# Jordy-VL/multi-modal-early-exit

Hardware: AMD Instinct MI355X
Metric: docs_per_sec (higher is better)
Workload: dtype f32 (operands split into 2 x f16, 3 f16 MFMA terms per MAC, f32 accumulate)

## Files before the change

include/mmee.h:

```cpp
#ifndef MMEE_H
#define MMEE_H

#include <stddef.h>
#include <stdint.h>

#ifdef __cplusplus
extern "C" {
#endif

#define MMEE_ABI_VERSION 4
#define MMEE_MAX_ENCODER_EXITS 64

enum { MMEE_EXIT_VISION_AVG = 0, MMEE_EXIT_TEXT_AVG = 1, MMEE_EXIT_TEXT_VISUAL_CONCAT = 2 };
enum { MMEE_STRATEGY_RAMP = 0, MMEE_STRATEGY_GATE = 1 };
enum { MMEE_CRIT_MAX_CONFIDENCE = 0, MMEE_CRIT_ENTROPY = 1, MMEE_CRIT_PATIENCE = 2, MMEE_CRIT_MARGIN = 3 };
enum { MMEE_RULE_PLAIN = 0, MMEE_RULE_STREAK = 1, MMEE_RULE_EITHER = 2 };
enum { MMEE_ARCH_LAYOUTLMV3 = 0, MMEE_ARCH_BEIT = 1 };
enum { MMEE_PREC_F32 = 0, MMEE_PREC_BF16 = 1, MMEE_PREC_F32_SPLIT = 2 };
enum { MMEE_DT_F32 = 0, MMEE_DT_F16 = 1, MMEE_DT_BF16 = 2 };
enum {
    MMEE_FLAG_DENSE_ROWS = 1,
    MMEE_FLAG_NO_EXIT = 2,
    MMEE_FLAG_WHOLE_LAYERS = 4,
    MMEE_FLAG_PROBE_ALWAYS = 8,
// ... 201 lines not shown
int ee_preprocess_images(const uint8_t* images, const void* desc, int32_t B, int32_t R, int32_t max_h, void* workspace,
                         size_t workspace_bytes, float* pixel_values, uint8_t* resized_u8, void* stream);
size_t ee_preprocess_workspace_bytes(int32_t B, int32_t R, int32_t max_h);
int ee_collate_pad(const int64_t* ids, const int64_t* boxes, const int64_t* offsets, int32_t B, int32_t T, int64_t pad_id,
                   int64_t* out_ids, int64_t* out_mask, int64_t* out_bbox, void* stream);

int ee_profile(ee_handle* h, int32_t enable);
int ee_profile_read(ee_handle* h, int32_t idx, char* name_out, int32_t name_cap, double* total_ms, int32_t* launches);

int ee_debug_gemm(const float* A, const float* W, const float* bias, const float* resid, float* Cout, int32_t M, int32_t N,
                  int32_t K, int32_t epi, int32_t wgs_per_cu, const int32_t* row_src, uint64_t* clk_probe, void* stream);

int ee_debug_gemm_split(const float* A, const float* W, const float* bias, const float* resid, float* Cout, int32_t M, int32_t N,
                        int32_t K, int32_t epi, int32_t out_split, float a_scale, float w_scale, float out_scale,
                        const int32_t* row_src, int32_t rows_A, int32_t iters, float* ms_out, void* stream);

#define MMEE_ATTN_KERNEL_F32 0
#define MMEE_ATTN_KERNEL_PAIR 1
#define MMEE_ATTN_KERNEL_IDX 2
#define MMEE_ATTN_KERNEL_IDX_NOBIAS 3
int ee_debug_attention(const float* qkv, int32_t qkv_rows, const int32_t* doc_off, int32_t n_docs, const int32_t* qkv_doc_off, const int32_t* pos,
                       const int32_t* x0, const int32_t* y1, const int32_t* masked, const float* w1, const float* wx, const float* wy, int32_t heads,
                       int32_t bins1, int32_t bins2, int32_t max_rel_pos, int32_t max_rel_2d_pos, int32_t max_pos, int32_t max_coord, int32_t kernel,
                       int32_t use_queue, int32_t q_limit, int32_t terms, void* ctx, int32_t* err_flag_out, void* stream);

typedef struct ee_debug_embed_args {
    const int64_t *input_ids, *attention_mask, *bbox, *position_ids, *token_type_ids;
    int32_t B, T, G, pad_id, vocab, max_2d, max_pos, type_vocab, dense_rows, H, cs, ss;
    const float *word, *type, *pos, *xtab, *ytab, *htab, *wtab, *inputs_embeds;
    const float *text_ln_g, *text_ln_b, *vis_ln_g, *vis_ln_b, *ln2_g, *ln2_b;
// ... 90 lines not shown
```

multi-modal-early-exit_amd/capi.py:

```python
from __future__ import annotations

import ctypes as C
import os
from typing import Optional

ABI_VERSION = 4
MAX_ENCODER_EXITS = 64
EXIT_KIND = {"vision_avg": 0, "text_avg": 1, "text_visual_concat": 2}
FLAG_DENSE_ROWS = 1
FLAG_NO_EXIT = 2
FLAG_WHOLE_LAYERS = 4
FLAG_PROBE_ALWAYS = 8
FLAG_XPROBE = 16
FLAG_ONE_TERM = 32
FLAG_LOW_LATENCY = 64
FLAG_STREAM_RESULTS = 128
CRIT_MAX_CONFIDENCE, CRIT_ENTROPY, CRIT_PATIENCE, CRIT_MARGIN = 0, 1, 2, 3
RULE_PLAIN, RULE_STREAK, RULE_EITHER = 0, 1, 2
SEARCH_GRID, SEARCH_SAMPLED, SEARCH_MIXTURES = 0, 1, 2
SEARCH_REFERENCE, SEARCH_POLICY = 0, 1
(METRIC_ACCURACY, METRIC_BRIER, METRIC_NLL, METRIC_F1_MICRO, METRIC_F1_MACRO, METRIC_ECE, METRIC_AURC, METRIC_AVG_CONF,
 METRIC_COUNT) = range(9)
DT_F32, DT_F16, DT_BF16 = 0, 1, 2
CLOCK_STAMP_WORDS = 4096
# ... 116 lines not shown
    "ee_rule_scan": (C.c_int, [_vp, C.c_double, _vp, _i32, _i32, _i32, C.POINTER(C.c_double), C.POINTER(_i32), _i32, _vp, _vp, _vp, _vp, _vp]),
    "ee_rule_sweep": (C.c_int, [_vp, _vp, _vp, _i32, _i32, _i32, _vp, _i32, C.POINTER(_i32), _i32, _i32, _vp, _vp, _vp, _vp]),
    "ee_patience_sweep": (C.c_int, [_vp, _vp, _i32, _i32, _i32, _vp, _i32, _vp, _vp, _vp, _vp]),
    "ee_pack_results": (C.c_int, [_vp, _vp, _vp, _i32, _i32, _vp, _vp]),
    "ee_unpack_results": (C.c_int, [_vp, _i32, _i32, _vp, _vp, _vp, _vp]),
    "ee_threshold_sweep": (C.c_int, [_vp, _vp, _i32, _i32, _vp, _i32, _vp, _vp, _vp, _vp]),
    "ee_threshold_search": (C.c_int, [_vp, _vp, _i32, _i32, _i32, _i32, C.c_int64, C.c_uint64, _vp, _i32, _vp, _vp, _vp, _vp, _vp, _vp, _vp, _vp, _vp]),
    "ee_threshold_search_cost": (C.c_int, [_vp, _vp, _vp, _i32, _i32, _i32, _i32, C.c_int64, C.c_uint64, _vp, _i32, _vp, _vp, _vp, _vp, _vp, _vp, _vp, _vp,
                                           _vp, _vp, _vp]),
    "ee_msp_table": (C.c_int, [_vp, _vp, _i32, _i32, _i32, _vp, _vp, _vp]),
    "ee_csf_table": (C.c_int, [_vp, _vp, _i32, _i32, _i32, _i32, _vp, _vp, _vp]),
    "ee_exit_metrics": (C.c_int, [_vp, _vp, _vp, _vp, _vp, _vp, _i32, _i32, _i32, _i32, _vp, _vp, _vp, _vp]),
    "ee_debug_gemm": (C.c_int, [_vp, _vp, _vp, _vp, _vp, _i32, _i32, _i32, _i32, _i32, _vp, _vp, _vp]),
    "ee_debug_gemm_split": (C.c_int, [_vp, _vp, _vp, _vp, _vp, _i32, _i32, _i32, _i32, _i32, C.c_float, C.c_float, C.c_float, _vp,
                                      _i32, _i32, C.POINTER(C.c_float), _vp]),
    "ee_debug_attn_stamps": (C.c_int, [_vp]),
    "ee_debug_attention": (C.c_int, [_vp, _i32, _vp, _i32, _vp, _vp, _vp, _vp, _vp, _vp, _vp, _vp, _i32, _i32, _i32, _i32, _i32, _i32, _i32, _i32,
                                     _i32, _i32, _i32, _vp, C.POINTER(_i32), _vp]),
    "ee_debug_prep": (C.c_int, [_vp, _vp, _vp, _vp, _vp, _i32, _i32, _i32, _i32, _i32, _i32, _i32, _i32, _i32, _vp, _vp, _vp, _vp, _vp, _vp, _vp, _vp,
                                C.POINTER(_i32), _vp]),
    "ee_debug_embed": (C.c_int, [C.POINTER(DebugEmbedArgs), C.POINTER(_i32), _vp]),
    "ee_debug_ln_rows": (C.c_int, [_vp, _vp, _vp, _vp, _i32, _i32, _vp, _vp, C.c_float, _vp, C.c_float, _i32, C.c_size_t, _vp, _vp, _vp, C.c_float,
                                   C.POINTER(_i32), _vp]),
    "ee_debug_xprobe": (C.c_int, [C.POINTER(DebugXProbeArgs), C.POINTER(_i32), _vp]),
    "ee_debug_head_out": (C.c_int, [C.POINTER(DebugHeadOutArgs), _vp]),
    "ee_debug_exit_decide": (C.c_int, [C.POINTER(DebugExitDecideArgs), _vp]),
    "ee_debug_rows_out": (C.c_int, [C.POINTER(DebugRowsOutArgs), _vp]),
    "ee_temperature_fit": (C.c_int, [_vp, _vp, _i32, _i32, _i32, _i32, _vp, _vp, _vp, _vp, _vp, _vp]),
    "ee_head_fit": (C.c_int, [_vp, _vp, _i32, _i32, _i32, _i32, C.c_double, C.c_double, _i32, _i32, _vp, C.c_size_t, _vp, _vp, _vp, _vp, _vp, _vp,
                              _vp, _vp, _vp]),
# ... 76 lines not shown
```

multi-modal-early-exit_amd/csrc/capi_tools.hip:

```cpp
#include <math.h>
#include <string.h>

#include <vector>

#include "capi_debug.h"

using namespace mmee;
using namespace mmee::capi;

namespace {

template <typename T>
struct TempUpload {
    T* dev = nullptr;
    hipStream_t s;
    const char* err = nullptr;
    TempUpload(const T* host, size_t n, hipStream_t stream) : s(stream) {
        if (hipMallocAsync((void**)&dev, sizeof(T) * n, s) != hipSuccess) { dev = nullptr; err = "hipMallocAsync failed"; }
        else if (hipMemcpyAsync(dev, host, sizeof(T) * n, hipMemcpyHostToDevice, s) != hipSuccess) err = "host-to-device copy failed";
    }
    TempUpload(const TempUpload&) = delete;
    ~TempUpload() { if (dev) (void)hipFreeAsync(dev, s); }
};

// ... 379 lines not shown
        launch_gemm_f32(g, epi, AMODE_ROWS, M, cus, reinterpret_cast<hipStream_t>(stream));
        set_gemm_wgs_per_cu(0);
    }
    return launch_status(nullptr, "ee_debug_gemm");
}

int ee_debug_attn_stamps(uint64_t* out8) {
    unsigned long long* d = mmee::attention_idx_stamps() ? mmee::attention_idx_stamps() : mmee::attention_pair_stamps();
    if (!out8 || !d) return fail(nullptr, "ee_debug_attn_stamps: no stamped launch has run (set MMEE_ATTN_STAMPS=1 before the first forward)");
    if (hipDeviceSynchronize() != hipSuccess || hipMemcpy(out8, d, 64, hipMemcpyDeviceToHost) != hipSuccess)
        return fail(nullptr, "ee_debug_attn_stamps: copy failed");
    (void)hipMemset(d, 0, 64);
    return 0;
}

int ee_debug_gemm_split(const float* A, const float* W, const float* bias, const float* resid, float* Cout, int32_t M, int32_t N,
                        int32_t K, int32_t epi, int32_t out_split, float a_scale, float w_scale, float out_scale,
                        const int32_t* row_src, int32_t rows_A, int32_t iters, float* ms_out, void* stream) {
    const int dbg = epi >> 4;
    epi &= 15;
#ifndef MMEE_DIAG
    if (dbg) return fail(nullptr, "ee_debug_gemm_split: timing variants (wrong results) exist in the diagnostic library only (make diag)");
#endif
    if (!A || !W || !Cout || M < 1 || rows_A < 1 || !mmee::gemm_split_supports(N, K) || epi < 0 || epi > 3 || iters < 1)
        return fail(nullptr, "ee_debug_gemm_split: bad argument (N %% 256, K %% 32)");
    if (epi == EPI_RESID && !resid) return fail(nullptr, "ee_debug_gemm_split: residual epilogue without a residual");
    hipStream_t s = reinterpret_cast<hipStream_t>(stream);
    const int cus = device_cus("ee_debug_gemm_split");
    if (!cus) return 1;
    float *As = nullptr, *Ws = nullptr;
    int* heads = nullptr;
    if (hipMalloc((void**)&As, (size_t)rows_A * K * 4) != hipSuccess || hipMalloc((void**)&Ws, (size_t)N * K * 4) != hipSuccess ||
        hipMalloc((void**)&heads, 512) != hipSuccess) {
        (void)hipFree(As); (void)hipFree(Ws); (void)hipFree(heads);
        return fail(nullptr, "ee_debug_gemm_split: hipMalloc failed");
    }
    mmee::launch_split_rows(A, As, nullptr, rows_A, rows_A, K, a_scale, cus, s);
    mmee::launch_split_rows(W, Ws, nullptr, N, N, K, w_scale, cus, s);
    GemmArgs g{};
    g.A = As; g.lda = K; g.W = Ws; g.bias = bias; g.C = Cout; g.ldc = N; g.resid = resid; g.ldr = N; g.m_static = M; g.N = N; g.K = K;
    g.scale = 1.f; g.alpha = 1.0f / (a_scale * w_scale); g.out_split = out_split ? 1 : 0; g.out_scale = out_scale;
    g.row_src = row_src; g.resid_row_src = row_src; g.tile_counter = heads; g.dbg_noload = dbg;
    unsigned long long* clk = nullptr;
    const int n_clk = 2 * 2 * cus;
    if (dbg && ms_out) {
        if (hipMalloc((void**)&clk, n_clk * 8) == hipSuccess) (void)hipMemsetAsync(clk, 0, n_clk * 8, s);
        g.clk_probe = clk;
    }
    hipEvent_t e0, e1;
    (void)hipEventCreate(&e0);
    (void)hipEventCreate(&e1);
    (void)hipMemsetAsync(heads, 0, 512, s);
    launch_gemm_split(g, epi, M, cus, s);
    (void)hipEventRecord(e0, s);
    for (int i = 1; i < iters; ++i) {
        (void)hipMemsetAsync(heads, 0, 512, s);
        launch_gemm_split(g, epi, M, cus, s);
// ... 3 lines not shown
    float ms = 0.f;
    if (iters > 1) (void)hipEventElapsedTime(&ms, e0, e1);
    if (ms_out) *ms_out = iters > 1 ? ms / (float)(iters - 1) : 0.f;
    if (clk) {
        std::vector<unsigned long long> hc(n_clk);
        (void)hipMemcpy(hc.data(), clk, n_clk * 8, hipMemcpyDeviceToHost);
        double sum = 0;
        int n = 0;
        for (int i = 0; i + 1 < n_clk; i += 2)
            if (hc[i + 1]) { sum += (double)hc[i] / (double)hc[i + 1] * 0.1; ++n; }
        ms_out[1] = n ? (float)(sum / n) : 0.f;
        (void)hipFree(clk);
    }
    (void)hipEventDestroy(e0);
    (void)hipEventDestroy(e1);
    (void)hipFree(As); (void)hipFree(Ws); (void)hipFree(heads);
    if (err != hipSuccess || hipGetLastError() != hipSuccess) return fail(nullptr, "ee_debug_gemm_split: launch failed: %s", hipGetErrorString(err));
    return 0;
}

}
```

multi-modal-early-exit_amd/csrc/gemm_split.hip:

```cpp
#include <cstdlib>
#include "mmee_common.h"

#include "gemm_split_kernel.h"

namespace mmee {

bool gemm_split_supports(int N, int K) { return N > 0 && K > 0 && N % 256 == 0 && K % 32 == 0; }

void launch_split_ffn_up(const GemmArgs& a, int max_m, int num_cus, hipStream_t s);

void launch_gemm_split(const GemmArgs& a_in, int epi, int max_m, int num_cus, hipStream_t s) {
    GemmArgs a = a_in;
    a.tile_order = a.N <= 768 ? 1 : 0;
    if (a.probe) a.terms = 3;
    if (a.probe) {
        if (a.out_split && epi == EPI_GELU) { launch_split_one<CfgP, EPI_GELU, true, false, 1>(a, max_m, num_cus, s); return; }
        if (!a.out_split && epi == EPI_RESID) { launch_split_one<CfgP, EPI_RESID, false, false, 1>(a, max_m, num_cus, s); return; }
        if (!a.out_split && epi == EPI_BIAS) { launch_split_one<CfgP, EPI_BIAS, false, false, 1>(a, max_m, num_cus, s); return; }
        if (!a.out_split && epi == EPI_TANH) { launch_split_one<CfgP, EPI_TANH, false, false, 1>(a, max_m, num_cus, s); return; }
    }
    if (a.k_splits > 1 && !a.out_split && epi == EPI_BIAS && a.terms != 1) {
        a.tile_counter = nullptr;
        launch_split_one<CfgP, EPI_BIAS, false, false, 1>(a, max_m, num_cus, s);
        return;
    }
    a.k_splits = 1;
    if (a.terms != 1 && (long)((max_m + 255) / 256) * (a.N / 256) * 2 <= (long)num_cus) {
        a.tile_counter = nullptr;
        if (a.out_split && epi == EPI_GELU) { launch_split_one<CfgP, EPI_GELU, true, false, 1>(a, max_m, num_cus, s); return; }
        if (a.out_split && epi == EPI_BIAS) { launch_split_one<CfgP, EPI_BIAS, true, false, 1>(a, max_m, num_cus, s); return; }
        if (!a.out_split && epi == EPI_RESID) { launch_split_one<CfgP, EPI_RESID, false, false, 1>(a, max_m, num_cus, s); return; }
        if (!a.out_split && epi == EPI_BIAS) { launch_split_one<CfgP, EPI_BIAS, false, false, 1>(a, max_m, num_cus, s); return; }
        if (!a.out_split && epi == EPI_TANH) { launch_split_one<CfgP, EPI_TANH, false, false, 1>(a, max_m, num_cus, s); return; }
        a.tile_counter = a_in.tile_counter;
    }
#ifdef MMEE_DIAG
    static const int order_env = diag_env_int("MMEE_GEMM_ORDER", -1);
    if (order_env == 0 || order_env == 1) a.tile_order = order_env;
    else if (order_env == 2) a.tile_order = a.N <= 768 ? 1 : 0;
    else if (order_env == 3 || order_env == 4) a.tile_order = a.N >= 2304 ? order_env - 1 : a.tile_order;
    static const int forced = diag_env_int("MMEE_SPLIT_CFG", 0);
    const bool use_a = forced == 1;
// ... 132 lines not shown
```

multi-modal-early-exit_amd/csrc/gemm_split_kernel.h:

```cpp
#pragma once
#include <cstdlib>
#include "mmee_common.h"

namespace mmee {


template <int BM_, int BN_, int ROWB_, int NST_, int WM_, int WN_, int WGS_, int MF_ = 32>
struct SplitCfg {
    static constexpr int BM = BM_, BN = BN_, ROWB = ROWB_, NST = NST_, WM = WM_, WN = WN_, WGS = WGS_;
    static constexpr int MF = MF_;
    static_assert(MF == 32 || (MF == 16 && ROWB == 128), "the 16x16x32 MFMA consumes one 128-byte row (k = 32) per step");
    static constexpr int NW = WM * WN, THREADS = NW * 64;
    static constexpr int KSTAGE = ROWB / 4;
    static constexpr int PROWS = 1024 / ROWB;
    static constexpr int PA = BM / PROWS / NW, PW = BN / PROWS / NW;
    static constexpr int PP = PA + PW;
    static constexpr int A_BYTES = BM * ROWB, STAGE_BYTES = (BM + BN) * ROWB, LOOP_BYTES = NST * STAGE_BYTES;
    static constexpr int EPI_BYTES = NW * 32 * 64 * 4;
    static_assert(BM == WM * 64 && BN == WN * 64, "one 64x64 sub-tile per wave");
    static_assert(PA * PROWS * NW == BM && PW * PROWS * NW == BN && PA >= 1 && PW >= 1, "DMA pieces must tile the stage");
    static_assert(EPI_BYTES <= LOOP_BYTES, "epilogue staging must fit in the stage ring");
    static_assert(NST >= 2 && NST <= 4, "ring depth");
    static_assert(THREADS <= 1024, "a workgroup is at most 16 waves");
    static_assert(WGS * (LOOP_BYTES + 16) <= 160 * 1024, "LDS budget of a CU (160 KiB) for WGS workgroups");
    static_assert(WGS * NW <= 32, "wave slots of a CU");
};
using CfgA = SplitCfg<128, 256, 64, 3, 2, 4, 2>;
using CfgB = SplitCfg<256, 256, 128, 2, 4, 4, 1>;
using CfgC = SplitCfg<256, 256, 128, 2, 4, 4, 1, 16>;
using CfgP = SplitCfg<128, 128, 128, 3, 2, 2, 1, 16>;


__device__ __forceinline__ void dma_piece(unsigned voff, unsigned long long base, unsigned lds_addr) {
    unsigned keep;
    asm volatile("s_mov_b32 %0, m0\n\ts_mov_b32 m0, %2\n\ts_nop 0\n\tglobal_load_lds_dwordx4 %1, %3\n\ts_mov_b32 m0, %0"
                 : "=&s"(keep)
                 : "v"(voff), "s"(lds_addr), "s"(base)
                 : "memory");
}

template <int EPI, bool OUT_SPLIT, int WN>
__device__ __forceinline__ void split_store_tile(const GemmArgs& g, float* smem, f32x16 (&acc)[2][2], int m0, int n0, int M,
                                                 int wave, int lane) {
    const int wr = wave / WN, wc = wave % WN;
    const int l31 = lane & 31, hh = lane >> 5;
    float* stg = smem + wave * (32 * 64);
    const int c4 = (lane & 15) * 4;
    const int col = n0 + wc * 64 + c4;
    f32x4 bv = f32x4{0.f, 0.f, 0.f, 0.f};
    if (g.bias) bv = *reinterpret_cast<const f32x4*>(g.bias + col);
    const float sc = (col < g.scale_cols) ? g.scale : 1.0f;
    f32x4 lam = f32x4{1.f, 1.f, 1.f, 1.f};
    if (g.col_scale) lam = *reinterpret_cast<const f32x4*>(g.col_scale + col);
// ... 53 lines not shown
                    const int c0 = __builtin_amdgcn_mov_dpp(h2.x, 0xDD, 0xf, 0xf, true), c1 = __builtin_amdgcn_mov_dpp(h2.y, 0xDD, 0xf, 0xf, true);
                    const int d0 = __builtin_amdgcn_mov_dpp(l2.x, 0xDD, 0xf, 0xf, true), d1 = __builtin_amdgcn_mov_dpp(l2.y, 0xDD, 0xf, 0xf, true);
                    piece.x = take_lo ? b0 : a0;
                    piece.y = take_lo ? b1 : a1;
                    piece.z = take_lo ? d0 : c0;
                    piece.w = take_lo ? d1 : c1;
                }
                if (row < M)
                    *reinterpret_cast<int4*>(reinterpret_cast<char*>(g.C) + (size_t)row * g.ldc * 4 + (size_t)(col >> 4) * 64 + (lane & 3) * 16) = piece;
            }
        }
    }
    if (OUT_SPLIT) split_flag_overflow(amax, g.err_flag);
}

template <int EPI, bool OUT_SPLIT, int WN, int RB>
__device__ __forceinline__ void split_store_tile16(const GemmArgs& g, float* smem, f32x4 (&acc)[4][4], int m0, int n0, int M,
                                                   int wave, int lane, const f32x4 bv, const f32x4 lam, const size_t c_shift = 0) {
    const int wr = wave / WN, wc = wave % WN;
    const int l15 = lane & 15, gq = lane >> 4;
    float* stg = smem + wave * (RB * 64);
    const int c4 = (lane & 15) * 4;
    const int col = n0 + wc * 64 + c4;
    const float sc = (col < g.scale_cols) ? g.scale : 1.0f;
    const float s_out = OUT_SPLIT ? g.out_scale : 1.0f;
    constexpr bool ACT = EPI == EPI_GELU || EPI == EPI_TANH;
    const bool sc_p2 = (__float_as_uint(sc) & 0x007fffffu) == 0u;
    const float fold = ACT ? 1.0f : s_out * (sc_p2 ? sc : 1.0f);
    const float post = ACT ? sc : (sc_p2 ? 1.0f : sc);
    const bool need_post = __builtin_amdgcn_readfirstlane((int)__float_as_uint(post)) != 0x3f800000;
    const bool need_lam = g.col_scale != nullptr;
    const float alpha_e = g.alpha * fold;
    const f32x4 be = bv * fold;
// ... 4 lines not shown
#pragma unroll
        for (int m2 = 0; m2 < RB / 16; ++m2)
#pragma unroll
            for (int ni = 0; ni < 4; ++ni)
#pragma unroll
                for (int e = 0; e < 4; ++e) {
                    const int r = 16 * m2 + 4 * gq + e;
                    stg[r * 64 + ((ni * 16 + l15) ^ (16 * (gq & 1)))] = acc[(RB / 16) * half + m2][ni][e];
                }
        asm volatile("" ::: "memory");
        const int rbase = m0 + wr * 64 + half * RB + (lane >> 4);
#pragma unroll
        for (int j = 0; j < RB / 4; ++j) {
            const int rl = (lane >> 4) + 4 * j;
            const int row = rbase + 4 * j;
            f32x4 v = *reinterpret_cast<const f32x4*>(stg + rl * 64 + (c4 ^ (16 * ((rl >> 2) & 1))));
#pragma unroll
            for (int t = 0; t < 4; t += 2) {
                f32x2 x = __builtin_elementwise_fma(f32x2{v[t], v[t + 1]}, (f32x2)(alpha_e), f32x2{be[t], be[t + 1]});
                if (need_post) x = x * (f32x2)(post);
                if (EPI == EPI_GELU) x = gelu_scaled2(x, gelu_c0, gelu_hs);
                if (EPI == EPI_TANH) { x[0] = tanhf(x[0]) * s_out; x[1] = tanhf(x[1]) * s_out; }
                if (need_lam) x = x * f32x2{lam[t], lam[t + 1]};
                v[t] = x[0];
                v[t + 1] = x[1];
            }
            if (row < M) {
                if (EPI == EPI_RESID) {
                    const int rs = g.resid_row_src ? g.resid_row_src[row] : row;
                    if (g.resid_split_inv != 0.f) {
                        const f32x4 r = load_split4_sum(g.resid + (size_t)rs * g.ldr, col);
#pragma unroll
                        for (int t = 0; t < 4; t += 2) {
                            const f32x2 y = __builtin_elementwise_fma(f32x2{r[t], r[t + 1]}, (f32x2)(g.resid_split_inv), f32x2{v[t], v[t + 1]});
                            v[t] = y[0];
                            v[t + 1] = y[1];
                        }
                    } else {
                        v += *reinterpret_cast<const f32x4*>(g.resid + (size_t)rs * g.ldr + col);
                    }
                }
                if (!OUT_SPLIT) *reinterpret_cast<f32x4*>(g.C + c_shift + (size_t)row * g.ldc + col) = v;
            }
// ... 60 lines not shown
    const int swz_even = ROWB == 64 ? ((p_row >> 2) & 3) : ((p_row >> 1) & 7);
    const unsigned chunk_even = 16u * (unsigned)(p_chunk ^ swz_even);
    const unsigned chunk_odd = ROWB == 64 ? chunk_even : 16u * (unsigned)(p_chunk ^ ((swz_even + 4) & 7));
    const unsigned rswz = ROWB == 64 ? (unsigned)((l31 >> 2) & 3) : (unsigned)((l31 >> 1) & 7);
    const unsigned a_row = (unsigned)(wr * 64 + l31) * ROWB;
    const unsigned w_row = (unsigned)A_BYTES + (unsigned)(wc * 64 + l31) * ROWB;
    const int l15 = lane & 15, lq = lane >> 4;
    const unsigned swz16 = (unsigned)((l15 >> 1) & 7);
    const unsigned c16_hi = 16u * (((unsigned)(lq & 1) + 4u * (unsigned)(lq >> 1)) ^ swz16);
    const unsigned c16_lo = 16u * (((unsigned)(lq & 1) + 4u * (unsigned)(lq >> 1) + 2u) ^ swz16);
    const unsigned a_row16 = (unsigned)(wr * 64 + l15) * ROWB;
    const unsigned w_row16 = (unsigned)A_BYTES + (unsigned)(wc * 64 + l15) * ROWB;
    const char* sbytes = reinterpret_cast<const char*>(smem);

    constexpr bool HANDOVER = Cfg::MF == 16 && NST == 2 && Cfg::NW * 4096 <= STAGE_BYTES;

    auto pop = [&](int& tm, int& tn) __attribute__((always_inline)) -> bool {
        if (g.tile_counter) {
            while (q_try < 8) {
                const int q = (my_xcd + q_try) & 7;
                if (tid == 0) *q_slot = atomicAdd(g.tile_counter + 16 * q, 1);
                __syncthreads();
                const int j = *q_slot;
                __syncthreads();
                if (g.tile_order >= 2) {
                    const int gq = q < n_groups ? (n_groups - q + 7) / 8 : 0;
                    if (g.tile_order == 2) {
                        constexpr int CW = 4;
                        const int nfull = tiles_n / CW, per_cb = gq * GM * CW;
                        int cb, jj, w;
// ... 35 lines not shown
                    continue;
                }
                ++q_try;
            }
            return false;
        }
        if (tile >= n_tiles) return false;
        int t2 = tile;
        if (KSPLIT) { t2 = tile / ksp; ks_pop = tile - t2 * ksp; }
        tm = t2 / tiles_n;
        tn = t2 - tm * tiles_n;
        tile += gridDim.x;
        return true;
    };

    struct TileCtx {
        int m0, n0;
        int kt0;
        unsigned a_voff[PA], w_voff[PW];
        unsigned long long a_base, w_base;
    };
    auto setup = [&](int tm, int tn, TileCtx& t) __attribute__((always_inline)) {
        t.m0 = __builtin_amdgcn_readfirstlane(tm * BM);
        t.n0 = __builtin_amdgcn_readfirstlane(tn * BN);
        t.kt0 = KSPLIT ? __builtin_amdgcn_readfirstlane(ks_pop * nk) : 0;
        int first = g.row_src ? g.row_src[t.m0] : t.m0;
        if (DIAG && (dbg & 16)) first = 0;
#pragma unroll
        for (int j = 0; j < PA; ++j) {
            const int piece = wave + Cfg::NW * j;
            int ra = t.m0 + Cfg::PROWS * piece + p_row;
            ra = ra < M ? ra : M - 1;
            if (DIAG && (dbg & 16)) ra = Cfg::PROWS * piece + p_row;
            const int sa = g.row_src ? g.row_src[ra] : ra;
            t.a_voff[j] = (unsigned)(sa - first) * (unsigned)g.lda * 4u + ((piece & 1) ? chunk_odd : chunk_even);
        }
#pragma unroll
        for (int j = 0; j < PW; ++j) {
            const int piece = wave + Cfg::NW * j;
            t.w_voff[j] = (unsigned)(Cfg::PROWS * piece + p_row) * (unsigned)g.K * 4u + ((piece & 1) ? chunk_odd : chunk_even);
        }
        const unsigned long long a_base_v = (unsigned long long)(size_t)g.A + (unsigned long long)first * (unsigned)g.lda * 4ull;
        const unsigned long long w_base_v = (unsigned long long)(size_t)g.W + (unsigned long long)t.n0 * (unsigned)g.K * 4ull;
        t.a_base = ((unsigned long long)(unsigned)__builtin_amdgcn_readfirstlane((int)(a_base_v >> 32)) << 32) |
                   (unsigned)__builtin_amdgcn_readfirstlane((int)(a_base_v & 0xffffffffu));
        t.w_base = ((unsigned long long)(unsigned)__builtin_amdgcn_readfirstlane((int)(w_base_v >> 32)) << 32) |
                   (unsigned)__builtin_amdgcn_readfirstlane((int)(w_base_v & 0xffffffffu));
    };
    auto issue = [&](const TileCtx& t, int kt, int buf) __attribute__((always_inline)) {
        const unsigned long long koff = (unsigned long long)(kt + (KSPLIT ? t.kt0 : 0)) * (unsigned)ROWB;
        const unsigned dst = lds0 + (unsigned)buf * STAGE_BYTES + (unsigned)wave * 1024u;
#pragma unroll
        for (int j = 0; j < PA; ++j) dma_piece(t.a_voff[j], t.a_base + koff, dst + (unsigned)(Cfg::NW * j) * 1024u);
#pragma unroll
        for (int j = 0; j < PW; ++j) dma_piece(t.w_voff[j], t.w_base + koff, dst + A_BYTES + (unsigned)(Cfg::NW * j) * 1024u);
    };

    TileCtx cur;
    int buf0 = 0;
    {
        int tm, tn;
        if (!pop(tm, tn)) return;
// ... 28 lines not shown
                asm volatile("s_waitcnt vmcnt(0)" ::: "memory");
            } else if (dbg & 4) {
                asm volatile("s_barrier" ::: "memory");
            } else if (NST == 4 && kt + 2 < nk) {
                static_assert(NST != 4 || Cfg::PP == 8, "vmcnt immediate: two stages' pieces per wave");
                asm volatile("s_waitcnt vmcnt(16)\n\ts_barrier" ::: "memory");
            } else if (NST >= 3 && kt + 1 < nk) {
                static_assert(Cfg::PP == 3 || Cfg::PP == 4 || Cfg::PP == 8, "vmcnt immediate: one stage's pieces per wave");
                if (Cfg::PP == 3) asm volatile("s_waitcnt vmcnt(3)\n\ts_barrier" ::: "memory");
                else if (Cfg::PP == 4) asm volatile("s_waitcnt vmcnt(4)\n\ts_barrier" ::: "memory");
                else asm volatile("s_waitcnt vmcnt(8)\n\ts_barrier" ::: "memory");
            } else {
                asm volatile("s_waitcnt vmcnt(0)\n\ts_barrier" ::: "memory");
            }
            if (kt + NST - 1 < nk && !(dbg & 1)) issue(cur, kt + NST - 1, bufn);
            const char* sb = sbytes + buf * STAGE_BYTES;
            if constexpr (Cfg::MF == 16) {
                f16x8 ah[4], al[4];
#pragma unroll
                for (int i = 0; i < 4; ++i) {
                    ah[i] = *reinterpret_cast<const f16x8*>(sb + a_row16 + c16_hi + i * 16 * ROWB);
                    al[i] = *reinterpret_cast<const f16x8*>(sb + a_row16 + c16_lo + i * 16 * ROWB);
                }
#pragma unroll
                for (int j = 0; j < 4; ++j) {
                    const f16x8 wh = *reinterpret_cast<const f16x8*>(sb + w_row16 + c16_hi + j * 16 * ROWB);
                    const f16x8 wl = *reinterpret_cast<const f16x8*>(sb + w_row16 + c16_lo + j * 16 * ROWB);
                    if (TERMS == 3) {
#pragma unroll
                        for (int i = 0; i < 4; ++i) acc16[i][j] = __builtin_amdgcn_mfma_f32_16x16x32_f16(al[i], wh, acc16[i][j], 0, 0, 0);
// ... 36 lines not shown
            if (g.col_scale) lam = *reinterpret_cast<const f32x4*>(g.col_scale + col);
            asm volatile("s_waitcnt vmcnt(0)" : "+v"(bv), "+v"(lam) :: "memory");
        }
        TileCtx nxt;
        bool have;
        {
            int tm, tn;
            have = pop(tm, tn);
            if (have) setup(tm, tn, nxt);
        }
        const int last_slot = (buf0 + nk - 1) % NST;
        const int nbuf0 = HANDOVER ? (last_slot ^ 1) : 0;
        if (HANDOVER && have) issue(nxt, 0, nbuf0);
        if (!(dbg & 8)) {
            if constexpr (Cfg::MF == 16) {
                if constexpr (HANDOVER)
                    split_store_tile16<EPI, OUT_SPLIT, WN, 16>(g, smem + last_slot * (STAGE_BYTES / 4), acc16, m0, n0, M, wave, lane, bv, lam);
                else
                    split_store_tile16<EPI, OUT_SPLIT, WN, 32>(g, smem, acc16, m0, n0, M, wave, lane, bv, lam, c_shift);
            } else {
                split_store_tile<EPI, OUT_SPLIT, WN>(g, smem, acc, m0, n0, M, wave, lane);
            }
        }
        __syncthreads();
        if (!have) break;
        cur = nxt;
        buf0 = nbuf0;
        if (!HANDOVER) {
            issue(cur, 0, 0);
            if (NST >= 3 && nk > 1) issue(cur, 1, 1);
            if (NST >= 4 && nk > 2) issue(cur, 2, 2);
        }
    }
    if (DIAG && g.clk_probe && threadIdx.x == 0) {
        g.clk_probe[2 * blockIdx.x] = __builtin_amdgcn_s_memtime() - clk0;
        g.clk_probe[2 * blockIdx.x + 1] = __builtin_amdgcn_s_memrealtime() - rt0;
    }
}

template <typename Cfg, int EPI, bool OUT_SPLIT, bool DIAG = false, int TAG = 0, int TERMS = 3>
static void launch_split_one(const GemmArgs& a, int max_m, int num_cus, hipStream_t s) {
    const size_t lds = Cfg::LOOP_BYTES + 16;
    (void)ensure_dynamic_lds<&gemm_split_kernel<Cfg, EPI, OUT_SPLIT, DIAG, TAG, TERMS>>("gemm_split_kernel", (int)lds);
    const int tiles = ((max_m + Cfg::BM - 1) / Cfg::BM) * (a.N / Cfg::BN) * (TAG == 1 && a.k_splits > 1 ? a.k_splits : 1);
    int grid = Cfg::WGS * num_cus;
    if (grid > tiles) grid = tiles;
    if (grid < 1) grid = 1;
    hipLaunchKernelGGL((gemm_split_kernel<Cfg, EPI, OUT_SPLIT, DIAG, TAG, TERMS>), dim3(grid), dim3(Cfg::THREADS), lds, s, a);
}

}
```

multi-modal-early-exit_amd/csrc/mmee_common.h:

```cpp
#pragma once
#include <hip/hip_runtime.h>
#include <stdint.h>

#include <stdio.h>
#include <stdlib.h>
#include <atomic>
#include <mutex>

namespace mmee {

inline int diag_env_int(const char* name, int dflt) {
#ifdef MMEE_DIAG
    const char* e = getenv(name);
    return e ? atoi(e) : dflt;
#else
    (void)name;
    return dflt;
#endif
}

struct LdsOptInError {
    std::mutex mu;
    int code = 0;
    char what[192] = {0};
// ... 236 lines not shown
    split_pair(v[0] * scale, v[1] * scale, h01, l01, amax);
    split_pair(v[2] * scale, v[3] * scale, h23, l23, amax);
    const bool take_lo = (lane & 2) != 0;
    const int a0 = __builtin_amdgcn_mov_dpp((int)h01, 0x88, 0xf, 0xf, true), a1 = __builtin_amdgcn_mov_dpp((int)h23, 0x88, 0xf, 0xf, true);
    const int b0 = __builtin_amdgcn_mov_dpp((int)l01, 0x88, 0xf, 0xf, true), b1 = __builtin_amdgcn_mov_dpp((int)l23, 0x88, 0xf, 0xf, true);
    const int c0 = __builtin_amdgcn_mov_dpp((int)h01, 0xDD, 0xf, 0xf, true), c1 = __builtin_amdgcn_mov_dpp((int)h23, 0xDD, 0xf, 0xf, true);
    const int d0 = __builtin_amdgcn_mov_dpp((int)l01, 0xDD, 0xf, 0xf, true), d1 = __builtin_amdgcn_mov_dpp((int)l23, 0xDD, 0xf, 0xf, true);
    int4 piece;
    piece.x = take_lo ? b0 : a0;
    piece.y = take_lo ? b1 : a1;
    piece.z = take_lo ? d0 : c0;
    piece.w = take_lo ? d1 : c1;
    *reinterpret_cast<int4*>(reinterpret_cast<char*>(row_base) + (size_t)(col >> 4) * 64 + (lane & 3) * 16) = piece;
}
typedef unsigned u32x2_t __attribute__((ext_vector_type(2)));
__device__ __forceinline__ f32x4 load_split4_sum(const void* row_base, int col) {
    const char* p = reinterpret_cast<const char*>(row_base) + (col >> 4) * 64 + (col & 15) * 2;
    const u32x2_t hi = *reinterpret_cast<const u32x2_t*>(p), lo = *reinterpret_cast<const u32x2_t*>(p + 32);
    float r0, r1, r2, r3;
    asm("v_fma_mix_f32 %0, %4, 1.0, %6 op_sel:[0,0,0] op_sel_hi:[1,0,1]\n\t"
        "v_fma_mix_f32 %1, %4, 1.0, %6 op_sel:[1,0,1] op_sel_hi:[1,0,1]\n\t"
        "v_fma_mix_f32 %2, %5, 1.0, %7 op_sel:[0,0,0] op_sel_hi:[1,0,1]\n\t"
        "v_fma_mix_f32 %3, %5, 1.0, %7 op_sel:[1,0,1] op_sel_hi:[1,0,1]"
        : "=&v"(r0), "=&v"(r1), "=&v"(r2), "=&v"(r3)
        : "v"(hi[0]), "v"(hi[1]), "v"(lo[0]), "v"(lo[1]));
    return f32x4{r0, r1, r2, r3};
}
__device__ __forceinline__ f32x4 load_split4(const void* row_base, int col, float inv_scale) {
    return load_split4_sum(row_base, col) * inv_scale;
}
constexpr float kSplitScaleX = 16.0f;
constexpr float kSplitScaleCtx = 64.0f;
constexpr float kSplitScaleH1 = 16.0f;
constexpr float kSplitScaleQKV = 16.0f;

enum { EPI_BIAS = 0, EPI_GELU = 1, EPI_RESID = 2, EPI_TANH = 3 };
enum { AMODE_ROWS = 0, AMODE_IM2COL = 1 };

struct GemmArgs {
    const float* A;
    int lda;
// ... 10 lines not shown
    int m_static;
    int N, K;
    int scale_cols;
    float scale;
    const float* col_scale;
    int k_splits;
    size_t split_stride;
    const float* pix;
    int C_in, R, P, G;
    float alpha;
    int out_split;
    float out_scale;
    int use_dma;
    int probe;
    int role_tag;
    int tile_order;
    int prio_mode;
    int terms;
    int dbg_noload;
    int* tile_counter;
    unsigned long long* clk_probe;
    int* err_flag;
};

struct AttnArgs {
    const float* qkv;
    int ld;
    float* ctx;
    int ldc;
    const RowMeta* meta;
// ... 56 lines not shown
```

Before: 7272.

## Stage split residual through LDS via async DMA in GEMM epilogue

```diff
diff --git a/include/mmee.h b/include/mmee.h
--- a/include/mmee.h
+++ b/include/mmee.h
@@ -239,6 +239,10 @@
 int ee_debug_gemm_split(const float* A, const float* W, const float* bias, const float* resid, float* Cout, int32_t M, int32_t N,
                         int32_t K, int32_t epi, int32_t out_split, float a_scale, float w_scale, float out_scale,
                         const int32_t* row_src, int32_t rows_A, int32_t iters, float* ms_out, void* stream);
+
+int ee_debug_gemm_split_resid(const float* A, const float* W, const float* bias, const float* resid, float* Cout, int32_t M, int32_t N,
+                              int32_t K, float a_scale, float w_scale, float resid_scale, const int32_t* row_src, int32_t rows_A,
+                              const int32_t* resid_row_src, int32_t rows_resid, int32_t route, int32_t iters, float* ms_out, void* stream);
 
 #define MMEE_ATTN_KERNEL_F32 0
 #define MMEE_ATTN_KERNEL_PAIR 1
diff --git a/multi-modal-early-exit_amd/capi.py b/multi-modal-early-exit_amd/capi.py
--- a/multi-modal-early-exit_amd/capi.py
+++ b/multi-modal-early-exit_amd/capi.py
@@ -154,6 +154,8 @@
     "ee_debug_gemm": (C.c_int, [_vp, _vp, _vp, _vp, _vp, _i32, _i32, _i32, _i32, _i32, _vp, _vp, _vp]),
     "ee_debug_gemm_split": (C.c_int, [_vp, _vp, _vp, _vp, _vp, _i32, _i32, _i32, _i32, _i32, C.c_float, C.c_float, C.c_float, _vp,
                                       _i32, _i32, C.POINTER(C.c_float), _vp]),
+    "ee_debug_gemm_split_resid": (C.c_int, [_vp, _vp, _vp, _vp, _vp, _i32, _i32, _i32, C.c_float, C.c_float, C.c_float, _vp, _i32, _vp, _i32,
+                                            _i32, _i32, C.POINTER(C.c_float), _vp]),
     "ee_debug_attn_stamps": (C.c_int, [_vp]),
     "ee_debug_attention": (C.c_int, [_vp, _i32, _vp, _i32, _vp, _vp, _vp, _vp, _vp, _vp, _vp, _vp, _i32, _i32, _i32, _i32, _i32, _i32, _i32, _i32,
                                      _i32, _i32, _i32, _vp, C.POINTER(_i32), _vp]),
diff --git a/multi-modal-early-exit_amd/csrc/capi_tools.hip b/multi-modal-early-exit_amd/csrc/capi_tools.hip
--- a/multi-modal-early-exit_amd/csrc/capi_tools.hip
+++ b/multi-modal-early-exit_amd/csrc/capi_tools.hip
@@ -417,33 +417,27 @@
     return 0;
 }
 
-int ee_debug_gemm_split(const float* A, const float* W, const float* bias, const float* resid, float* Cout, int32_t M, int32_t N,
-                        int32_t K, int32_t epi, int32_t out_split, float a_scale, float w_scale, float out_scale,
-                        const int32_t* row_src, int32_t rows_A, int32_t iters, float* ms_out, void* stream) {
-    const int dbg = epi >> 4;
-    epi &= 15;
-#ifndef MMEE_DIAG
-    if (dbg) return fail(nullptr, "ee_debug_gemm_split: timing variants (wrong results) exist in the diagnostic library only (make diag)");
-#endif
-    if (!A || !W || !Cout || M < 1 || rows_A < 1 || !mmee::gemm_split_supports(N, K) || epi < 0 || epi > 3 || iters < 1)
-        return fail(nullptr, "ee_debug_gemm_split: bad argument (N %% 256, K %% 32)");
-    if (epi == EPI_RESID && !resid) return fail(nullptr, "ee_debug_gemm_split: residual epilogue without a residual");
-    hipStream_t s = reinterpret_cast<hipStream_t>(stream);
-    const int cus = device_cus("ee_debug_gemm_split");
+static int run_debug_gemm_split(const char* who, GemmArgs g, int epi, const float* A, const float* W, int rows_A, float a_scale, float w_scale,
+                                const float* resid, int rows_resid, float resid_scale, int M, int iters, float* ms_out, hipStream_t s) {
+    const int dbg = g.dbg_noload;
+    const int N = g.N, K = g.K;
+    const int cus = device_cus(who);
     if (!cus) return 1;
-    float *As = nullptr, *Ws = nullptr;
+    float *As = nullptr, *Ws = nullptr, *Rs = nullptr;
     int* heads = nullptr;
     if (hipMalloc((void**)&As, (size_t)rows_A * K * 4) != hipSuccess || hipMalloc((void**)&Ws, (size_t)N * K * 4) != hipSuccess ||
-        hipMalloc((void**)&heads, 512) != hipSuccess) {
-        (void)hipFree(As); (void)hipFree(Ws); (void)hipFree(heads);
-        return fail(nullptr, "ee_debug_gemm_split: hipMalloc failed");
+        hipMalloc((void**)&heads, 512) != hipSuccess ||
+        (resid_scale != 0.f && hipMalloc((void**)&Rs, (size_t)rows_resid * N * 4) != hipSuccess)) {
+        (void)hipFree(As); (void)hipFree(Ws); (void)hipFree(heads); (void)hipFree(Rs);
+        return fail(nullptr, "%s: hipMalloc failed", who);
     }
     mmee::launch_split_rows(A, As, nullptr, rows_A, rows_A, K, a_scale, cus, s);
     mmee::launch_split_rows(W, Ws, nullptr, N, N, K, w_scale, cus, s);
-    GemmArgs g{};
-    g.A = As; g.lda = K; g.W = Ws; g.bias = bias; g.C = Cout; g.ldc = N; g.resid = resid; g.ldr = N; g.m_static = M; g.N = N; g.K = K;
-    g.scale = 1.f; g.alpha = 1.0f / (a_scale * w_scale); g.out_split = out_split ? 1 : 0; g.out_scale = out_scale;
-    g.row_src = row_src; g.resid_row_src = row_src; g.tile_counter = heads; g.dbg_noload = dbg;
+    g.A = As; g.W = Ws; g.tile_counter = heads;
+    if (resid_scale != 0.f) {
+        mmee::launch_split_rows(resid, Rs, nullptr, rows_resid, rows_resid, N, resid_scale, cus, s);
+        g.resid = Rs; g.resid_split_inv = 1.0f / resid_scale;
+    }
     unsigned long long* clk = nullptr;
     const int n_clk = 2 * 2 * cus;
     if (dbg && ms_out) {
@@ -477,9 +471,55 @@
     }
     (void)hipEventDestroy(e0);
     (void)hipEventDestroy(e1);
-    (void)hipFree(As); (void)hipFree(Ws); (void)hipFree(heads);
-    if (err != hipSuccess || hipGetLastError() != hipSuccess) return fail(nullptr, "ee_debug_gemm_split: launch failed: %s", hipGetErrorString(err));
+    (void)hipFree(As); (void)hipFree(Ws); (void)hipFree(heads); (void)hipFree(Rs);
+    if (err != hipSuccess || hipGetLastError() != hipSuccess) return fail(nullptr, "%s: launch failed: %s", who, hipGetErrorString(err));
     return 0;
 }
 
-}
+int ee_debug_gemm_split(const float* A, const float* W, const float* bias, const float* resid, float* Cout, int32_t M, int32_t N,
+                        int32_t K, int32_t epi, int32_t out_split, float a_scale, float w_scale, float out_scale,
+                        const int32_t* row_src, int32_t rows_A, int32_t iters, float* ms_out, void* stream) {
+    const int dbg = epi >> 4;
+    epi &= 15;
+#ifndef MMEE_DIAG
+    if (dbg) return fail(nullptr, "ee_debug_gemm_split: timing variants (wrong results) exist in the diagnostic library only (make diag)");
+#endif
+    if (!A || !W || !Cout || M < 1 || rows_A < 1 || !mmee::gemm_split_supports(N, K) || epi < 0 || epi > 3 || iters < 1)
+        return fail(nullptr, "ee_debug_gemm_split: bad argument (N %% 256, K %% 32)");
+    if (epi == EPI_RESID && !resid) return fail(nullptr, "ee_debug_gemm_split: residual epilogue without a residual");
+    GemmArgs g{};
+    g.lda = K; g.bias = bias; g.C = Cout; g.ldc = N; g.resid = resid; g.ldr = N; g.m_static = M; g.N = N; g.K = K;
+    g.scale = 1.f; g.alpha = 1.0f / (a_scale * w_scale); g.out_split = out_split ? 1 : 0; g.out_scale = out_scale;
+    g.row_src = row_src; g.resid_row_src = row_src; g.dbg_noload = dbg;
+    return run_debug_gemm_split("ee_debug_gemm_split", g, epi, A, W, rows_A, a_scale, w_scale, nullptr, 0, 0.f, M, iters, ms_out,
+                                reinterpret_cast<hipStream_t>(stream));
+}
+
+static int check_row_map(const char* who, const char* what, const int32_t* map, int M, int rows) {
+    std::vector<int> h;
+    if (!to_host(h, map, (size_t)M)) return fail(nullptr, "%s: copy of %s failed", who, what);
+    for (int i = 0; i < M; ++i)
+        if (h[i] < 0 || h[i] >= rows) return fail(nullptr, "%s: %s[%d] = %d outside [0, %d)", who, what, i, h[i], rows);
+    return 0;
+}
+
+int ee_debug_gemm_split_resid(const float* A, const float* W, const float* bias, const float* resid, float* Cout, int32_t M, int32_t N,
+                              int32_t K, float a_scale, float w_scale, float resid_scale, const int32_t* row_src, int32_t rows_A,
+                              const int32_t* resid_row_src, int32_t rows_resid, int32_t route, int32_t iters, float* ms_out, void* stream) {
+    const char* who = "ee_debug_gemm_split_resid";
+    if (!A || !W || !resid || !Cout || M < 1 || rows_A < 1 || rows_resid < 1 || !mmee::gemm_split_supports(N, K) || iters < 1 || route < 0 ||
+        route > 2 || !(a_scale > 0.f) || !(w_scale > 0.f) || resid_scale < 0.f)
+        return fail(nullptr, "%s: bad argument (N %% 256, K %% 32, route 0 / 1 / 2)", who);
+    if ((!row_src && M > rows_A) || (!resid_row_src && M > rows_resid)) return fail(nullptr, "%s: M rows without a row map need M rows of A / of the residual", who);
+    if (row_src) { const int rc = check_row_map(who, "row_src", row_src, M, rows_A); if (rc) return rc; }
+    if (resid_row_src) { const int rc = check_row_map(who, "resid_row_src", resid_row_src, M, rows_resid); if (rc) return rc; }
+    GemmArgs g{};
+    g.lda = K; g.bias = bias; g.C = Cout; g.ldc = N; g.resid = resid; g.ldr = N; g.m_static = M; g.N = N; g.K = K;
+    g.scale = 1.f; g.alpha = 1.0f / (a_scale * w_scale);
+    g.row_src = row_src; g.resid_row_src = resid_row_src; g.route = route;
+    g.role_tag = K > N ? 3 : 2;
+    return run_debug_gemm_split(who, g, EPI_RESID, A, W, rows_A, a_scale, w_scale, resid, rows_resid, resid_scale, M, iters, ms_out,
+                                reinterpret_cast<hipStream_t>(stream));
+}
+
+}
diff --git a/multi-modal-early-exit_amd/csrc/gemm_split.hip b/multi-modal-early-exit_amd/csrc/gemm_split.hip
--- a/multi-modal-early-exit_amd/csrc/gemm_split.hip
+++ b/multi-modal-early-exit_amd/csrc/gemm_split.hip
@@ -25,7 +25,12 @@
         return;
     }
     a.k_splits = 1;
-    if (a.terms != 1 && (long)((max_m + 255) / 256) * (a.N / 256) * 2 <= (long)num_cus) {
+    if (a.route == 1 && !a.out_split && epi == EPI_RESID) {
+        a.tile_counter = nullptr;
+        launch_split_one<CfgP, EPI_RESID, false, false, 1>(a, max_m, num_cus, s);
+        return;
+    }
+    if (a.terms != 1 && a.route != 2 && (long)((max_m + 255) / 256) * (a.N / 256) * 2 <= (long)num_cus) {
         a.tile_counter = nullptr;
         if (a.out_split && epi == EPI_GELU) { launch_split_one<CfgP, EPI_GELU, true, false, 1>(a, max_m, num_cus, s); return; }
         if (a.out_split && epi == EPI_BIAS) { launch_split_one<CfgP, EPI_BIAS, true, false, 1>(a, max_m, num_cus, s); return; }
diff --git a/multi-modal-early-exit_amd/csrc/gemm_split_kernel.h b/multi-modal-early-exit_amd/csrc/gemm_split_kernel.h
--- a/multi-modal-early-exit_amd/csrc/gemm_split_kernel.h
+++ b/multi-modal-early-exit_amd/csrc/gemm_split_kernel.h
@@ -24,6 +24,7 @@
     static_assert(THREADS <= 1024, "a workgroup is at most 16 waves");
     static_assert(WGS * (LOOP_BYTES + 16) <= 160 * 1024, "LDS budget of a CU (160 KiB) for WGS workgroups");
     static_assert(WGS * NW <= 32, "wave slots of a CU");
+    static constexpr int RESID_OFF = LOOP_BYTES + 16, RESID_MAP_OFF = RESID_OFF + NW * 1024, RESID_BYTES = NW * (1024 + 2 * 256);
 };
 using CfgA = SplitCfg<128, 256, 64, 3, 2, 4, 2>;
 using CfgB = SplitCfg<256, 256, 128, 2, 4, 4, 1>;
@@ -37,6 +38,32 @@
                  : "=&s"(keep)
                  : "v"(voff), "s"(lds_addr), "s"(base)
                  : "memory");
+}
+
+__device__ __forceinline__ void dma_piece_addr(unsigned long long addr, unsigned lds_addr) {
+    unsigned keep;
+    asm volatile("s_mov_b32 %0, m0\n\ts_mov_b32 m0, %2\n\ts_nop 0\n\tglobal_load_lds_dwordx4 %1, off\n\ts_mov_b32 m0, %0"
+                 : "=&s"(keep)
+                 : "v"(addr), "s"(lds_addr)
+                 : "memory");
+}
+
+template <typename Cfg, int EPI, bool OUT_SPLIT, bool DIAG>
+constexpr bool resid_lds_staged() {
+    return Cfg::MF == 16 && Cfg::NST == 2 && Cfg::NW * 4096 <= Cfg::STAGE_BYTES && Cfg::BM == 256 && EPI == EPI_RESID && !OUT_SPLIT && !DIAG;
+}
+struct ResidStage {
+    const int* rmap;
+    unsigned long long base;
+    unsigned ldr4;
+    unsigned d_lds, s_lds;
+    const char* d_ptr;
+};
+__device__ __forceinline__ void resid_piece_issue(const ResidStage& rs, int g, unsigned lds_addr, int lane) {
+    asm volatile("" : "+v"(lane));
+    const int src = rs.rmap[4 * g + (lane >> 4)];
+    const unsigned chunk = 16u * (unsigned)((lane & 15) ^ (2 * ((lane >> 4) & 1)));
+    dma_piece_addr(rs.base + (unsigned long long)(unsigned)src * rs.ldr4 + chunk, lds_addr);
 }
 
 template <int EPI, bool OUT_SPLIT, int WN>
@@ -120,9 +147,11 @@
     if (OUT_SPLIT) split_flag_overflow(amax, g.err_flag);
 }
 
-template <int EPI, bool OUT_SPLIT, int WN, int RB>
+template <int EPI, bool OUT_SPLIT, int WN, int RB, bool RSTG = false>
 __device__ __forceinline__ void split_store_tile16(const GemmArgs& g, float* smem, f32x4 (&acc)[4][4], int m0, int n0, int M,
-                                                   int wave, int lane, const f32x4 bv, const f32x4 lam, const size_t c_shift = 0) {
+                                                   int wave, int lane, const f32x4 bv, const f32x4 lam, const size_t c_shift = 0,
+                                                   const ResidStage* rst = nullptr) {
+    static_assert(!RSTG || (EPI == EPI_RESID && !OUT_SPLIT && RB == 16), "the staged residual: 16-row slices, f32 output");
     const int wr = wave / WN, wc = wave % WN;
     const int l15 = lane & 15, gq = lane >> 4;
     float* stg = smem + wave * (RB * 64);
@@ -157,7 +186,34 @@
         for (int j = 0; j < RB / 4; ++j) {
             const int rl = (lane >> 4) + 4 * j;
             const int row = rbase + 4 * j;
+            u32x2_t rhi = u32x2_t{0u, 0u}, rlo = u32x2_t{0u, 0u};
+            if constexpr (RSTG) {
+                const int gp = 4 * half + j;
+                if (gp > 0) {
+                    if ((j & 2) && gp != 15) asm volatile("s_waitcnt vmcnt(3)" ::: "memory");
+                    else asm volatile("s_waitcnt vmcnt(2)" ::: "memory");
+                }
+                const char* slot = (j & 1) ? reinterpret_cast<const char*>(stg) + (j >> 1) * 1024 : rst->d_ptr;
+                int ln = lane;
+                asm volatile("" : "+v"(ln));
+                const unsigned hi_off = (unsigned)(ln >> 4) * 256u + (unsigned)((ln & 15) >> 2) * 64u +
+                                        (((unsigned)(ln & 3) * 8u) ^ (32u * (unsigned)((ln >> 4) & 1)));
+                rhi = *reinterpret_cast<const u32x2_t*>(slot + hi_off);
+                rlo = *reinterpret_cast<const u32x2_t*>(slot + (hi_off ^ 32u));
+            }
             f32x4 v = *reinterpret_cast<const f32x4*>(stg + rl * 64 + (c4 ^ (16 * ((rl >> 2) & 1))));
+            if constexpr (RSTG) {
+                asm volatile("s_waitcnt lgkmcnt(0)" : "+v"(rhi), "+v"(rlo), "+v"(v) :: "memory");
+                const int gp = 4 * half + j;
+                if (j == 0) {
+                    resid_piece_issue(*rst, gp + 1, rst->s_lds, lane);
+                    resid_piece_issue(*rst, gp + 2, rst->d_lds, lane);
+                } else if (j == 1) {
+                    resid_piece_issue(*rst, gp + 2, rst->s_lds + 1024u, lane);
+                } else if (j == 2 && gp + 2 < 16) {
+                    resid_piece_issue(*rst, gp + 2, rst->d_lds, lane);
+                }
+            }
 #pragma unroll
             for (int t = 0; t < 4; t += 2) {
                 f32x2 x = __builtin_elementwise_fma(f32x2{v[t], v[t + 1]}, (f32x2)(alpha_e), f32x2{be[t], be[t + 1]});
@@ -168,8 +224,17 @@
                 v[t] = x[0];
                 v[t + 1] = x[1];
             }
+            if constexpr (RSTG) {
+                const f32x4 r = split4_sum(rhi, rlo);
+#pragma unroll
+                for (int t = 0; t < 4; t += 2) {
+                    const f32x2 y = __builtin_elementwise_fma(f32x2{r[t], r[t + 1]}, (f32x2)(g.resid_split_inv), f32x2{v[t], v[t + 1]});
+                    v[t] = y[0];
+                    v[t + 1] = y[1];
+                }
+            }
             if (row < M) {
-                if (EPI == EPI_RESID) {
+                if (EPI == EPI_RESID && !RSTG) {
                     const int rs = g.resid_row_src ? g.resid_row_src[row] : row;
                     if (g.resid_split_inv != 0.f) {
                         const f32x4 r = load_split4_sum(g.resid + (size_t)rs * g.ldr, col);
@@ -260,6 +325,10 @@
     const char* sbytes = reinterpret_cast<const char*>(smem);
 
     constexpr bool HANDOVER = Cfg::MF == 16 && NST == 2 && Cfg::NW * 4096 <= STAGE_BYTES;
+    constexpr bool RSTG = resid_lds_staged<Cfg, EPI, OUT_SPLIT, DIAG>();
+    static_assert(!RSTG || (HANDOVER && (Cfg::RESID_OFF + Cfg::RESID_BYTES + 1279) / 1280 * 1280 <= 160 * 1024),
+                  "the staged residual needs the 4 KiB staging blocks of the hand-over and its slots inside the CU's 160 KiB of LDS");
+    const bool rstg = RSTG && g.resid_split_inv != 0.f;
 
     auto pop = [&](int& tm, int& tn) __attribute__((always_inline)) -> bool {
         if (g.tile_counter) {
@@ -325,22 +394,44 @@
         return true;
     };
 
+    int rpar_next = 0;
+    auto rmap_of = [&](int par) __attribute__((always_inline)) -> int* {
+        return reinterpret_cast<int*>(reinterpret_cast<char*>(smem) + Cfg::RESID_MAP_OFF + (wave * 2 + par) * 256);
+    };
     struct TileCtx {
         int m0, n0;
         int kt0;
         unsigned a_voff[PA], w_voff[PW];
         unsigned long long a_base, w_base;
+        int rpar;
     };
     auto setup = [&](int tm, int tn, TileCtx& t) __attribute__((always_inline)) {
         t.m0 = __builtin_amdgcn_readfirstlane(tm * BM);
         t.n0 = __builtin_amdgcn_readfirstlane(tn * BN);
         t.kt0 = KSPLIT ? __builtin_amdgcn_readfirstlane(ks_pop * nk) : 0;
+        t.rpar = rpar_next;
+        if constexpr (RSTG) {
+            if (rstg) {
+                int ln = lane;
+                asm volatile("" : "+v"(ln));
+                int rr = t.m0 + wr * 64 + ln;
+                rr = rr < M ? rr : M - 1;
+                rmap_of(t.rpar)[ln] = g.resid_row_src ? g.resid_row_src[rr] : rr;
+                rpar_next ^= 1;
+            }
+        }
         int first = g.row_src ? g.row_src[t.m0] : t.m0;
+        int p_row_s = p_row;
+        if constexpr (RSTG) {
+            int ln = lane;
+            asm volatile("" : "+v"(ln));
+            p_row_s = ln / CPR;
+        }
         if (DIAG && (dbg & 16)) first = 0;
 #pragma unroll
         for (int j = 0; j < PA; ++j) {
             const int piece = wave + Cfg::NW * j;
-            int ra = t.m0 + Cfg::PROWS * piece + p_row;
+            int ra = t.m0 + Cfg::PROWS * piece + p_row_s;
             ra = ra < M ? ra : M - 1;
             if (DIAG && (dbg & 16)) ra = Cfg::PROWS * piece + p_row;
             const int sa = g.row_src ? g.row_src[ra] : ra;
@@ -357,6 +448,16 @@
                    (unsigned)__builtin_amdgcn_readfirstlane((int)(a_base_v & 0xffffffffu));
         t.w_base = ((unsigned long long)(unsigned)__builtin_amdgcn_readfirstlane((int)(w_base_v >> 32)) << 32) |
                    (unsigned)__builtin_amdgcn_readfirstlane((int)(w_base_v & 0xffffffffu));
+    };
+    auto resid_stage = [&](const TileCtx& t) __attribute__((always_inline)) -> ResidStage {
+        ResidStage r;
+        r.rmap = rmap_of(t.rpar);
+        r.base = (unsigned long long)(size_t)g.resid + (unsigned long long)(unsigned)(t.n0 + wc * 64) * 4ull;
+        r.ldr4 = (unsigned)g.ldr * 4u;
+        r.d_lds = lds0 + (unsigned)Cfg::RESID_OFF + (unsigned)wave * 1024u;
+        r.s_lds = 0;
+        r.d_ptr = sbytes + Cfg::RESID_OFF + wave * 1024;
+        return r;
     };
     auto issue = [&](const TileCtx& t, int kt, int buf) __attribute__((always_inline)) {
         const unsigned long long koff = (unsigned long long)(kt + (KSPLIT ? t.kt0 : 0)) * (unsigned)ROWB;
@@ -415,6 +516,12 @@
                 asm volatile("s_waitcnt vmcnt(0)\n\ts_barrier" ::: "memory");
             }
             if (kt + NST - 1 < nk && !(dbg & 1)) issue(cur, kt + NST - 1, bufn);
+            if constexpr (RSTG) {
+                if (rstg && kt == nk - 1) {
+                    const ResidStage r0 = resid_stage(cur);
+                    resid_piece_issue(r0, 0, r0.d_lds, lane);
+                }
+            }
             const char* sb = sbytes + buf * STAGE_BYTES;
             if constexpr (Cfg::MF == 16) {
                 f16x8 ah[4], al[4];
@@ -481,7 +588,12 @@
         if (HANDOVER && have) issue(nxt, 0, nbuf0);
         if (!(dbg & 8)) {
             if constexpr (Cfg::MF == 16) {
-                if constexpr (HANDOVER)
+                if constexpr (RSTG) {
+                    ResidStage rst = resid_stage(cur);
+                    rst.s_lds = lds0 + (unsigned)last_slot * STAGE_BYTES + (unsigned)wave * 4096u;
+                    if (rstg) split_store_tile16<EPI, OUT_SPLIT, WN, 16, true>(g, smem + last_slot * (STAGE_BYTES / 4), acc16, m0, n0, M, wave, lane, bv, lam, 0, &rst);
+                    else split_store_tile16<EPI, OUT_SPLIT, WN, 16>(g, smem + last_slot * (STAGE_BYTES / 4), acc16, m0, n0, M, wave, lane, bv, lam);
+                } else if constexpr (HANDOVER)
                     split_store_tile16<EPI, OUT_SPLIT, WN, 16>(g, smem + last_slot * (STAGE_BYTES / 4), acc16, m0, n0, M, wave, lane, bv, lam);
                 else
                     split_store_tile16<EPI, OUT_SPLIT, WN, 32>(g, smem, acc16, m0, n0, M, wave, lane, bv, lam, c_shift);
@@ -507,7 +619,7 @@
 
 template <typename Cfg, int EPI, bool OUT_SPLIT, bool DIAG = false, int TAG = 0, int TERMS = 3>
 static void launch_split_one(const GemmArgs& a, int max_m, int num_cus, hipStream_t s) {
-    const size_t lds = Cfg::LOOP_BYTES + 16;
+    const size_t lds = Cfg::LOOP_BYTES + 16 + (resid_lds_staged<Cfg, EPI, OUT_SPLIT, DIAG>() ? Cfg::RESID_BYTES : 0);
     (void)ensure_dynamic_lds<&gemm_split_kernel<Cfg, EPI, OUT_SPLIT, DIAG, TAG, TERMS>>("gemm_split_kernel", (int)lds);
     const int tiles = ((max_m + Cfg::BM - 1) / Cfg::BM) * (a.N / Cfg::BN) * (TAG == 1 && a.k_splits > 1 ? a.k_splits : 1);
     int grid = Cfg::WGS * num_cus;
diff --git a/multi-modal-early-exit_amd/csrc/mmee_common.h b/multi-modal-early-exit_amd/csrc/mmee_common.h
--- a/multi-modal-early-exit_amd/csrc/mmee_common.h
+++ b/multi-modal-early-exit_amd/csrc/mmee_common.h
@@ -274,9 +274,7 @@
     *reinterpret_cast<int4*>(reinterpret_cast<char*>(row_base) + (size_t)(col >> 4) * 64 + (lane & 3) * 16) = piece;
 }
 typedef unsigned u32x2_t __attribute__((ext_vector_type(2)));
-__device__ __forceinline__ f32x4 load_split4_sum(const void* row_base, int col) {
-    const char* p = reinterpret_cast<const char*>(row_base) + (col >> 4) * 64 + (col & 15) * 2;
-    const u32x2_t hi = *reinterpret_cast<const u32x2_t*>(p), lo = *reinterpret_cast<const u32x2_t*>(p + 32);
+__device__ __forceinline__ f32x4 split4_sum(const u32x2_t hi, const u32x2_t lo) {
     float r0, r1, r2, r3;
     asm("v_fma_mix_f32 %0, %4, 1.0, %6 op_sel:[0,0,0] op_sel_hi:[1,0,1]\n\t"
         "v_fma_mix_f32 %1, %4, 1.0, %6 op_sel:[1,0,1] op_sel_hi:[1,0,1]\n\t"
@@ -285,6 +283,10 @@
         : "=&v"(r0), "=&v"(r1), "=&v"(r2), "=&v"(r3)
         : "v"(hi[0]), "v"(hi[1]), "v"(lo[0]), "v"(lo[1]));
     return f32x4{r0, r1, r2, r3};
+}
+__device__ __forceinline__ f32x4 load_split4_sum(const void* row_base, int col) {
+    const char* p = reinterpret_cast<const char*>(row_base) + (col >> 4) * 64 + (col & 15) * 2;
+    return split4_sum(*reinterpret_cast<const u32x2_t*>(p), *reinterpret_cast<const u32x2_t*>(p + 32));
 }
 __device__ __forceinline__ f32x4 load_split4(const void* row_base, int col, float inv_scale) {
     return load_split4_sum(row_base, col) * inv_scale;
@@ -325,6 +327,7 @@
     int use_dma;
     int probe;
     int role_tag;
+    int route;
     int tile_order;
     int prio_mode;
     int terms;
```

Measured after the change: 7352, median of 6. +1.1%, better.
